# wzhe06/SparrowRecSys

Hardware: AMD Instinct MI355X
Metric: ctr_samples_per_sec (higher is better)
Workload: dtype f32

## Files before the change

sparrowrecsys_amd/csrc/host_setup_common.h:

```cpp
struct DinVariant { int kc, hc, max_t; };
const DinVariant kDinVariants[] = {{2, 2, 64}, {1, 2, 64}};

int fold_first_dense(sprk_engine* h, DevPlan* dp) {
    if (!h->tune.tile_fold) return SPRK_OK;
    if (dp->n_ops < 1) return SPRK_OK;
    DevOp& op = dp->ops[0];
    if (op.kind != SPRK_OP_DENSE || op.src_buf != 0 || op.dst_buf == 0 || op.N > 512) return SPRK_OK;
    const int lo0 = op.src_off, hi0 = op.src_off + op.K;
    auto used_elsewhere = [&](int a, int b) {
        std::vector<char> live(b - a, 1);
        auto reads = [&](int s0, int s1) {
            for (int c = (s0 > a ? s0 : a); c < (s1 < b ? s1 : b); ++c) if (live[c - a]) return true;
            return false;
        };
        auto writes = [&](int s0, int s1) { for (int c = (s0 > a ? s0 : a); c < (s1 < b ? s1 : b); ++c) live[c - a] = 0; };
        for (int i = 1; i < dp->n_ops; ++i) {
            const DevOp& o = dp->ops[i];
            if (o.src_buf == 0) {
                if (o.kind == SPRK_OP_PAIR_DOT) {
                    for (int p = 0; p < dp->n_pairs; ++p)
                        if (reads(dp->pair_a[p], dp->pair_a[p] + o.K) || reads(dp->pair_b[p], dp->pair_b[p] + o.K)) return true;
                } else if (o.kind == SPRK_OP_FM_SUMSQ) {
                    if (reads(o.src_off, o.src_off + (o.groups - 1) * o.group_stride + o.K)) return true;
                } else if (reads(o.src_off, o.src_off + o.K)) {
// ... 60 lines not shown
        std::vector<DevSeg> plain, acc;
        for (int i = 0; i < dp->n_segs; ++i) (dp->segs[i].kind == SEG_ROWS_ACC ? acc : plain).push_back(dp->segs[i]);
        int k = 0;
        for (const DevSeg& g : plain) dp->segs[k++] = g;
        for (const DevSeg& g : acc) dp->segs[k++] = g;
        dp->n_acc = (int)acc.size();
        h->n_acc_folded = dp->n_acc;
    }
    op.W = wcopy + (lo - lo0);
    op.src_off = lo;
    op.K = hi - lo;
    op.acc_init = 1;
    return SPRK_OK;
}

int wide_dynamic_range(const float* rows, long long nrows, int row_floats, int ncols, float mx, bool* wide) {
    *wide = false;
    const bool guard_on = g_finalize_tune ? g_finalize_tune->half_range_guard : SprkTuning::from_env().half_range_guard;
    if (!guard_on || !(mx > 0.f) || nrows <= 0) return SPRK_OK;
    DevScratch<unsigned long long> d_cnt;
    HIP_TRY(d_cnt.alloc(2));
    HIP_TRY(hipMemset(d_cnt.p, 0, 2 * sizeof(unsigned long long)));
    long long blocks = (nrows * ncols + 255) / 256;
    if (blocks > 8192) blocks = 8192;
    hipLaunchKernelGGL(k_v2_count_small, dim3((unsigned)blocks), dim3(256), 0, 0, rows, nrows, row_floats, ncols, ldexpf(mx, -20), d_cnt.p);
    HIP_TRY(hipGetLastError());
    unsigned long long cnt[2] = {0, 0};
    HIP_TRY(hipMemcpy(cnt, d_cnt.p, sizeof(cnt), hipMemcpyDeviceToHost));
    *wide = cnt[0] * 1024ull > cnt[1];
    return SPRK_OK;
}

inline float absmax_nan(float m, float v) { const float a = fabsf(v); return (a > m || a != a) ? a : m; }
bool wide_dynamic_range_host(const float* v, size_t n, float mx) {
    const bool guard_on = g_finalize_tune ? g_finalize_tune->half_range_guard : SprkTuning::from_env().half_range_guard;
    if (!guard_on || !(mx > 0.f)) return false;
    const float thresh = ldexpf(mx, -20);
    unsigned long long small = 0, nz = 0;
    for (size_t i = 0; i < n; ++i) {
        const float a = fabsf(v[i]);
// ... 13 lines not shown

struct AbsmaxJob { const float* x; long long rows; int row_floats, ncols; unsigned grid; int slot; };
int device_absmax(const std::vector<AbsmaxJob>& jobs, float* mx, int n_out) {
    DevScratch<unsigned> d_max;
    HIP_TRY(d_max.alloc(n_out));
    HIP_TRY(hipMemset(d_max.p, 0, n_out * sizeof(unsigned)));
    for (const AbsmaxJob& j : jobs)
        hipLaunchKernelGGL(k_v2_absmax, dim3(j.grid), dim3(256), 0, 0, j.x, j.rows, j.row_floats, j.ncols, d_max.p + j.slot);
    HIP_TRY(hipGetLastError());
    static_assert(sizeof(unsigned) == sizeof(float), "k_v2_absmax keeps float bits in an unsigned word");
    HIP_TRY(hipMemcpy(mx, d_max.p, n_out * sizeof(float), hipMemcpyDeviceToHost));
    return SPRK_OK;
}
unsigned absmax_grid(long long n, long long cap) { const long long b = (n + 255) / 256; return (unsigned)(b < cap ? b : cap); }

int static_scale(const std::vector<AbsmaxJob>& tabs, float* scale, float* mx_out = nullptr) {
    *scale = 0.f;
    float mx = 0.f;
    SPRK_TRY(device_absmax(tabs, &mx, 1));
    if (mx_out) *mx_out = mx;
    if (!(mx < 3.0e38f)) return SPRK_OK;
    for (const AbsmaxJob& t : tabs) {
        bool wide = false;
        SPRK_TRY(wide_dynamic_range(t.x, t.rows, t.row_floats, t.ncols, mx, &wide));
        if (wide) return SPRK_OK;
    }
    *scale = pow2_scale(mx);
    return SPRK_OK;
}
float static_scale_host(const float* v, size_t n) {
    float mx = 0.f;
    for (size_t i = 0; i < n; ++i) mx = absmax_nan(mx, v[i]);
    if (!(mx < 3.0e38f) || wide_dynamic_range_host(v, n, mx)) return 0.f;
    return pow2_scale(mx);
}

int make_dyn_fragments(sprk_engine* h, const float* W, int ld, int N, int K, float** frag, float* w_scale_out, int kvalid = -1) {
    *frag = nullptr;
    if (kvalid < 0) kvalid = K;
// ... 15 lines not shown
```

sparrowrecsys_amd/csrc/host_setup_v2.h:

```cpp
constexpr int V2_WAVES = 8;
struct V2Variant {
    int g_emb, kpc, h0c, h1c;
    size_t lds_bytes;
    void (*pack)(const V2Args, float*);
};
#define V2_LDS(G_EMB, DV, KPC, H0C, H1C, FOLD) \
    (sizeof(float) * (V2Lds<G_EMB, DV, KPC, H0C, H1C, FOLD>::total_pad + V2_WAVES * V2Lds<G_EMB, DV, KPC, H0C, H1C, FOLD>::stage_floats))
#define V2_VARIANT(G_EMB) {G_EMB, 1, 2, 1, V2_LDS(G_EMB, 4, 1, 2, 1, true), &k_v2_pack_image<G_EMB, 4, 1, 2, 1, true>}
const V2Variant kV2Variants[] = {
    V2_VARIANT(6),
    V2_VARIANT(4),
    V2_VARIANT(5), V2_VARIANT(3), V2_VARIANT(2),
};

struct V2JVariant {
    int g_big, njf, kpc;
    bool half;
    V2JKernel fn;
    V2JManyKernel fn_many;
    V2JManyTabKernel fn_many_tab;
};
#define V2J_VARIANT(G_BIG, NJF, HALF) \
    {G_BIG, NJF, 1, HALF, &k_deepfm_v2_joint<G_BIG, NJF, 1, 2, 1, V2_WAVES, HALF>, &k_deepfm_v2_joint_many<G_BIG, NJF, 1, 2, 1, V2_WAVES, HALF>, \
     &k_deepfm_v2_joint_many_tab<G_BIG, NJF, 1, 2, 1, V2_WAVES, HALF>}
// ... 140 lines not shown
}

int setup_v2_joint(sprk_engine* h) {
    const V2Variant& vv = kV2Variants[h->v2_variant];
    if (vv.kpc != 1 || vv.h0c != 2 || vv.h1c != 1 || !h->tune.v2_joint) return SPRK_OK;
    const int KP = 16, H0 = 32, G = vv.g_emb;
    int big[V2_MAX_FIELDS], nbig = 0, jf[V2_MAX_FIELDS], njf = 0;
    for (int g = 0; g < G; ++g) {
        const long long v1 = (long long)h->v2run.vocab[g] + 1;
        if (v1 <= 32 && njf < V2J_MAX_JF) jf[njf++] = g;
        else big[nbig++] = g;
    }
    if (njf < 1 || nbig < 1 || nbig > 3) return SPRK_OK;
    bool half = h->tune.v2_half;
    float p_scale = 1.f, w_scale = 1.f;
    if (half) {
        std::vector<AbsmaxJob> rows_jobs;
        for (int b = 0; b < nbig; ++b) {
            const long long rows = (long long)h->v2run.vocab[big[b]] + 1;
            rows_jobs.push_back({h->v2_folded + (size_t)h->v2run.rowbase[big[b]] * (KP + 16), rows, KP + 16, KP, absmax_grid(rows * KP, 8192), 0});
        }
        SPRK_TRY(static_scale(rows_jobs, &p_scale));
        if (p_scale != 0.f) SPRK_TRY(static_scale({{h->v2.W0, (long long)H0, (G + 1) * KP, (G + 1) * KP, 8, 0}}, &w_scale));
        if (p_scale == 0.f || w_scale == 0.f) { half = false; p_scale = w_scale = 1.f; }
    }
    int variant = -1;
    for (size_t v = 0; v < sizeof(kV2JVariants) / sizeof(kV2JVariants[0]); ++v)
        if (kV2JVariants[v].g_big == nbig && kV2JVariants[v].njf == njf && kV2JVariants[v].half == half) variant = (int)v;
    if (variant < 0) return SPRK_OK;
    V2JRun& r = h->v2j_run;
    memset(&r, 0, sizeof(r));
    r.F = h->v2run.F; r.ND = h->v2run.ND; r.n_num = h->v2run.n_num;
    r.h0w = h->v2run.h0w; r.fo_bias = h->v2run.fo_bias; r.head_bias = h->v2run.head_bias;
    for (int b = 0; b < nbig; ++b) {
        r.big_col[b] = h->v2run.col[big[b]]; r.big_vocab[b] = h->v2run.vocab[big[b]];
        r.big_rowbase[b] = h->v2run.rowbase[big[b]]; r.big_grp[b] = big[b];
    }
    size_t small_floats = 0;
    for (int f = 0; f < njf; ++f) {
// ... 9 lines not shown
    for (int f = 0; f < njf; ++f) {
        const int rows = r.j_vocab[f] + 1;
        hipLaunchKernelGGL(k_v2_fold_small, dim3((rows + 3) / 4), dim3(256), 0, 0,
                           h->v2_folded + (size_t)h->v2run.rowbase[jf[f]] * (KP + 16), KP, H0, jf[f], h->v2.W0, (G + 1) * KP,
                           h->v2.b0, f == 0 ? 1 : 0, h->v2j_tab + r.s_off[f], rows);
    }
    if (half)
        hipLaunchKernelGGL(k_v2j_fold_num, dim3(8), dim3(256), 0, 0, h->v2.W0, (G + 1) * KP, G * KP, h->v2.Wp[G], h->v2.ldp_num,
                           h->v2.bp[G], h->v2.n_num, KP, H0, h->v2j_tab + r.wf_off, h->v2j_tab + r.s_off[0], r.j_vocab[0] + 1);
    HIP_TRY(hipGetLastError());
    HIP_TRY(hipDeviceSynchronize());
    r.small_floats = (int)small_floats;
    r.tab0 = h->v2_folded;
    r.small = h->v2j_tab;
    r.w_scale = w_scale; r.unscale_h = 1.f / (p_scale * w_scale); r.unscale_s = 1.f / p_scale;
    if (half) {
        size_t big_rows = 0;
        for (int b = 0; b < nbig; ++b) big_rows += (size_t)r.big_vocab[b] + 1;
        if (big_rows * (KP + 16) * sizeof(float) >= ((size_t)1 << 32)) return fail(SPRK_EINVAL, "split rows exceed 32-bit offsets");
        SPRK_TRY(table_alloc(h, &h->v2j_big, big_rows * (KP + 16) * sizeof(float)));
        h->derived_bytes += big_rows * (KP + 16) * sizeof(float);
        size_t base = 0;
        for (int b = 0; b < nbig; ++b) {
            const long long rows = (long long)r.big_vocab[b] + 1;
            long long nb = (rows * 8 + 255) / 256;
            if (nb > 65536) nb = 65536;
            hipLaunchKernelGGL(k_v2_split_rows, dim3((unsigned)nb), dim3(256), 0, 0,
                               h->v2_folded + (size_t)r.big_rowbase[b] * (KP + 16), h->v2j_big + base * (KP + 16), rows, p_scale);
            r.big_rowbase[b] = (unsigned)base;
            base += (size_t)rows;
        }
        HIP_TRY(hipGetLastError());
        HIP_TRY(hipDeviceSynchronize());
        r.tab0 = h->v2j_big;
    }
    h->v2j_lds_bytes = vv.lds_bytes + small_floats * sizeof(float);
    SPRK_TRY(set_max_lds(kV2JVariants[variant].fn, h->v2j_lds_bytes));
    SPRK_TRY(set_max_lds(kV2JVariants[variant].fn_many, h->v2j_lds_bytes));
    SPRK_TRY(set_max_lds(kV2JVariants[variant].fn_many_tab, h->v2j_lds_bytes));
    h->v2j_variant = variant;
    if (half && h->tune.v2j_one) {
        for (size_t v = 0; v < sizeof(kV2J1Variants) / sizeof(kV2J1Variants[0]); ++v) {
            const V2J1Variant& ov = kV2J1Variants[v];
// ... 55 lines not shown
```

sparrowrecsys_amd/csrc/k_chain_v2j.h:

```cpp

#define V2J_MAX_BIG 4
#define V2J_MAX_JF 3
#define V2J_SS 52

struct V2JRun {
    int F, ND, n_num;
    int big_col[V2J_MAX_BIG];
    int big_vocab[V2J_MAX_BIG];
    unsigned big_rowbase[V2J_MAX_BIG];
    int big_grp[V2J_MAX_BIG];
    int j_col[V2J_MAX_JF];
    int j_vocab[V2J_MAX_JF];
    int s_off[V2J_MAX_JF];
    int small_floats;
    int wf_off;
    const float* tab0;
    const float* small;
    float h0w, fo_bias, head_bias;
    int flags;
    float w_scale, unscale_h, unscale_s;
};

#define V2J_MB 64
struct V2JMany {
    const int* ids[V2J_MB];
    const float* dense[V2J_MB];
    float* out[V2J_MB];
    int n;
    int ntpb;
};
struct V2JBatch {
    const int* ids;
    const float* dense;
    float* out;
    void* pad_;
};
struct V2JManyTab {
    const V2JBatch* batch;
    int n;
    int ntpb;
};
struct V2JOne {};
__device__ __forceinline__ const int* v2j_ids(const V2JMany& m, int b) { return m.ids[b]; }
__device__ __forceinline__ const float* v2j_dense(const V2JMany& m, int b) { return m.dense[b]; }
__device__ __forceinline__ float* v2j_out(const V2JMany& m, int b) { return m.out[b]; }
typedef const __attribute__((address_space(4))) V2JBatch* V2JBatchCP;
__device__ __forceinline__ const int* v2j_ids(const V2JManyTab& m, int b) { return ((V2JBatchCP)(uintptr_t)m.batch + b)->ids; }
__device__ __forceinline__ const float* v2j_dense(const V2JManyTab& m, int b) { return ((V2JBatchCP)(uintptr_t)m.batch + b)->dense; }
__device__ __forceinline__ float* v2j_out(const V2JManyTab& m, int b) { return ((V2JBatchCP)(uintptr_t)m.batch + b)->out; }

__device__ __forceinline__ void split_half4(f32x4 w, float scale, f16x4& hi, f16x4& lo) {
#pragma unroll
    for (int j = 0; j < 4; ++j) {
        const float x = w[j] * scale;
        const _Float16 h = (_Float16)x;
        hi[j] = h;
        lo[j] = (_Float16)(x - (float)h);
    }
}

static __global__ __launch_bounds__(256) void k_v2_absmax(const float* __restrict__ rows, long long nrows, int row_floats,
                                                   int ncols, unsigned* __restrict__ out) {
    float m = 0.f;
    const long long total = nrows * ncols;
    for (long long i = (long long)blockIdx.x * 256 + threadIdx.x; i < total; i += (long long)gridDim.x * 256) {
// ... 8 lines not shown
static __global__ __launch_bounds__(256) void k_v2_count_small(const float* __restrict__ rows, long long nrows, int row_floats, int ncols,
                                                        float thresh, unsigned long long* __restrict__ out) {
    unsigned small = 0, nz = 0;
    const long long total = nrows * ncols;
    for (long long i = (long long)blockIdx.x * 256 + threadIdx.x; i < total; i += (long long)gridDim.x * 256) {
        const long long v = i / ncols;
        const int c = (int)(i - v * ncols);
        const float a = fabsf(rows[v * row_floats + c]);
        nz += a > 0.f;
        small += (a > 0.f && a < thresh);
    }
    for (int d = 32; d >= 1; d >>= 1) { small += __shfl_xor(small, d); nz += __shfl_xor(nz, d); }
    if ((threadIdx.x & 63) == 0) { atomicAdd(out, (unsigned long long)small); atomicAdd(out + 1, (unsigned long long)nz); }
}
static __global__ __launch_bounds__(256) void k_v2_split_rows(const float* __restrict__ src, float* __restrict__ dst,
                                                       long long nrows, float scale) {
    const long long total = nrows * 8;
    for (long long i = (long long)blockIdx.x * 256 + threadIdx.x; i < total; i += (long long)gridDim.x * 256) {
        const long long v = i >> 3;
        const int pc = (int)(i & 7);
        const f32x4 in = ld4(src + v * 32 + 4 * pc);
        if (pc < 4) {
            f16x4 hi, lo;
            split_half4(in, scale, hi, lo);
            f16x8 o = {hi[0], hi[1], hi[2], hi[3], lo[0], lo[1], lo[2], lo[3]};
            *reinterpret_cast<f16x8*>(dst + v * 32 + 4 * pc) = o;
        } else {
            st4(dst + v * 32 + 4 * pc, in);
        }
    }
}

static __global__ __launch_bounds__(256) void k_v2_fold_small(const float* __restrict__ folded, int KP, int H0, int grp,
                                                       const float* __restrict__ W0, int ldw0,
                                                       const float* __restrict__ b0, int add_b0,
                                                       float* __restrict__ out, int rows) {
    const int FS = KP + 16;
    for (int v = blockIdx.x * 4 + (threadIdx.x >> 6); v < rows; v += gridDim.x * 4) {
        const int col = threadIdx.x & 63;
        const float* prow = folded + (size_t)v * FS;
        float acc = 0.f;
        if (col < KP) {
            acc = prow[col];
        } else if (col < KP + H0) {
// ... 44 lines not shown
    int so[NJF];
    f32x4 xn;
    float w1a;
    float* dst;
};

template <int G_BIG, int NJF, int KPC, int H0C, int H1C, int WAVES, bool HALF, class Many>
__device__ __forceinline__ void v2j_body(const V2JRun& A, const int* __restrict__ ids, const float* __restrict__ dense,
                                         float* __restrict__ out, int B, int* __restrict__ err,
                                         const float* __restrict__ image, const Many* __restrict__ Mp) {
    constexpr bool MB = !std::is_same<Many, V2JOne>::value;
    constexpr int G_EMB = G_BIG + NJF;
    using LD = V2Lds<G_EMB, 4, KPC, H0C, H1C, true>;
    using Set = V2JSet<G_BIG, NJF>;
    constexpr int KP = LD::KP, H0 = H0C * 16;
    constexpr unsigned RB = (KP + 16) * 4;
    static_assert(KP + H0 + 1 <= V2J_SS, "small-field row layout");
    constexpr int NKR = HALF ? 1 : (G_BIG + 1) * KPC;
    static_assert(KPC == 1, "row layout: one 16-float chunk of projections per field");
    static_assert(G_BIG >= 1 && G_BIG <= 3 && NJF >= 1 && NJF <= V2J_MAX_JF, "field split");
    const int tid = threadIdx.x;
    const int lane = tid & 63;
    const int wave = __builtin_amdgcn_readfirstlane(tid >> 6);
    const int r = lane & 15, q = lane >> 4;
    const f32x4 zero = f32x4{0.f, 0.f, 0.f, 0.f};
    int m_ntpb = 0, ntasks = (B + 15) >> 4;
    if constexpr (MB) { m_ntpb = Mp->ntpb; ntasks = Mp->n * m_ntpb; }
    const int task_stride = gridDim.x * WAVES;
    const int wave_global = blockIdx.x * WAVES + wave;
    auto batch_of = [&](int tk) -> int {
        if constexpr (MB) return __builtin_amdgcn_readfirstlane(tk / m_ntpb);
// ... 54 lines not shown
            const float* nrow = stage + 128 + r * A.ND;
            const int c0 = 4 * q, last = A.n_num - 1;
            if constexpr (HALF) {
                S.xn.x = nrow[min(q, last)];
                S.xn.y = nrow[min(q + 4, last)];
            } else {
                S.xn.x = nrow[min(c0 + 0, last)];
                S.xn.y = nrow[min(c0 + 1, last)];
                S.xn.z = nrow[min(c0 + 2, last)];
                S.xn.w = nrow[min(c0 + 3, last)];
            }
        }
        const char* tb = reinterpret_cast<const char*>(A.tab0);
#pragma unroll
        for (int b = 0; b < G_BIG; ++b) S.x[b] = *reinterpret_cast<const f32x4*>(tb + (sid[b] * RB + 16u * q));
        {
            unsigned s0 = sid[0] * RB, s1 = sid[G_BIG > 1 ? 1 : 0] * RB, s2 = sid[G_BIG > 2 ? 2 : 0] * RB;
            asm("" : "+v"(s0), "+v"(s1), "+v"(s2));
            unsigned so = s0;
            if (G_BIG > 1) so = q == 1 ? s1 : so;
            if (G_BIG > 2) so = q == 2 ? s2 : so;
            S.w1a = *reinterpret_cast<const float*>(tb + (so + 4u * KP));
        }
        {
            float* out_b;
            if constexpr (MB) {
                out_b = v2j_out(*Mp, b);
                asm("" : "+s"(out_b));
            } else {
                out_b = out;
            }
            const int m = tk * 16 + r;
            S.dst = (q == 0 && m < B) ? out_b + m : nullptr;
        }
    };

    f32x4 rW0[H0C][NKR], rW1[H1C][H0C];
    f32x4 rwn[KPC], rbpn[KPC], rb1[H1C], rhfm[KPC], rhd[H1C];
    f32x4 rfn = zero;
    float rwn8[2] = {0.f, 0.f}, rfn8[2] = {0.f, 0.f}, rwf[H0C][2];
    f16x8 hWa[HALF ? G_BIG : 1][H0C], hWb[HALF ? G_BIG : 1][H0C];
    f16x8 hSel = {0, 0, 0, 0, 0, 0, 0, 0};
    auto load_weights = [&]() {
        const float* w0r = wq + LD::off_w0 + r * LD::S0;
#pragma unroll
        for (int n0 = 0; n0 < H0C; ++n0) {
            if constexpr (HALF) {
                rwf[n0][0] = small_s[A.wf_off + (n0 * 16 + r) * 8 + q];
                rwf[n0][1] = small_s[A.wf_off + (n0 * 16 + r) * 8 + q + 4];
            } else {
                rW0[n0][0] = ld4(w0r + n0 * 16 * LD::S0 + 16 * G_EMB);
            }
#pragma unroll
            for (int b = 0; b < G_BIG; ++b) {
                const f32x4 w = ld4(w0r + n0 * 16 * LD::S0 + 16 * A.big_grp[b]);
// ... 18 lines not shown
            rb1[n1] = ld4(wq + LD::off_b1 + n1 * 16);
            rhd[n1] = ld4(wq + LD::off_hd + n1 * 16);
        }
#pragma unroll
        for (int nb = 0; nb < KPC; ++nb) {
            rwn[nb] = ld4(wq + LD::off_wn + (nb * 16 + r) * LD::SN);
            rbpn[nb] = ld4(wq + LD::off_bp + G_EMB * KP + nb * 16);
            rhfm[nb] = ld4(wq + LD::off_hfm + nb * 16);
        }
        rfn = ld4(smem + LD::off_fn + 4 * (q & 1));
        if constexpr (HALF) {
            rwn8[0] = smem[LD::off_wn + r * LD::SN + q];
            rwn8[1] = smem[LD::off_wn + r * LD::SN + q + 4];
            rfn8[0] = smem[LD::off_fn + q];
            rfn8[1] = smem[LD::off_fn + q + 4];
        }
    };

    auto compute = [&](const Set& S) -> float {
#pragma clang fp contract(off)
        const f32x4 pnum = S.xn;
        f32x4 pn;
        if constexpr (HALF) {
            const f32x4 e = __builtin_amdgcn_mfma_f32_16x16x4f32(rwn8[0], pnum.x, rbpn[0], 0, 0, 0);
            const f32x4 o = __builtin_amdgcn_mfma_f32_16x16x4f32(rwn8[1], pnum.y, zero, 0, 0, 0);
            pn = e + o;
        } else {
            f32x4 e = rbpn[0], o = zero;
            e = __builtin_amdgcn_mfma_f32_16x16x4f32(rwn[0].x, pnum.x, e, 0, 0, 0);
            o = __builtin_amdgcn_mfma_f32_16x16x4f32(rwn[0].y, pnum.y, o, 0, 0, 0);
            e = __builtin_amdgcn_mfma_f32_16x16x4f32(rwn[0].z, pnum.z, e, 0, 0, 0);
            o = __builtin_amdgcn_mfma_f32_16x16x4f32(rwn[0].w, pnum.w, o, 0, 0, 0);
            pn = e + o;
        }
        float zz = ((q < G_BIG) ? S.w1a : 0.f) + (HALF ? __builtin_fmaf(rfn8[1], pnum.y, rfn8[0] * pnum.x) : ((q < 2) ? dot4f(rfn, pnum) : 0.f));
        f32x4 sp = ld4(small_s + S.so[0] + 4 * q), sq[H0C];
#pragma unroll
        for (int n0 = 0; n0 < H0C; ++n0) sq[n0] = ld4(small_s + S.so[0] + KP + 16 * n0 + 4 * q);
        float ssc = small_s[S.so[0] + KP + H0];
#pragma unroll
        for (int f = 1; f < NJF; ++f) {
            sp += ld4(small_s + S.so[f] + 4 * q);
#pragma unroll
            for (int n0 = 0; n0 < H0C; ++n0) sq[n0] += ld4(small_s + S.so[f] + KP + 16 * n0 + 4 * q);
            ssc += small_s[S.so[f] + KP + H0];
        }
        zz += (q == 3) ? ssc : 0.f;
        f32x4 hA[H0C], hB[H0C];
#pragma unroll
        for (int n0 = 0; n0 < H0C; ++n0) { hA[n0] = sq[n0]; hB[n0] = zero; }
        f32x4 s = sp + pn;
        if constexpr (HALF) {
            f32x4 aFa[H0C], aFb[H0C], aS = zero;
#pragma unroll
            for (int n0 = 0; n0 < H0C; ++n0) { aFa[n0] = zero; aFb[n0] = zero; }
            __builtin_amdgcn_sched_barrier(0);
#pragma unroll
            for (int b = 0; b < G_BIG; ++b) {
                const f16x8 xb = __builtin_bit_cast(f16x8, S.x[b]);
#pragma unroll
                for (int n0 = 0; n0 < H0C; ++n0) aFa[n0] = __builtin_amdgcn_mfma_f32_16x16x32_f16(hWa[b][n0], xb, aFa[n0], 0, 0, 0);
                aS = __builtin_amdgcn_mfma_f32_16x16x32_f16(hSel, xb, aS, 0, 0, 0);
#pragma unroll
                for (int n0 = 0; n0 < H0C; ++n0) aFb[n0] = __builtin_amdgcn_mfma_f32_16x16x32_f16(hWb[b][n0], xb, aFb[n0], 0, 0, 0);
                __builtin_amdgcn_sched_barrier(0);
            }
#pragma unroll
            for (int st = 0; st < 2; ++st)
#pragma unroll
                for (int n0 = 0; n0 < H0C; ++n0)
                    hA[n0] = __builtin_amdgcn_mfma_f32_16x16x4f32(rwf[n0][st], st ? pnum.y : pnum.x, hA[n0], 0, 0, 0);
            s = fma4s(aS, A.unscale_s, s);
#pragma unroll
            for (int n0 = 0; n0 < H0C; ++n0) hB[n0] = (aFa[n0] + aFb[n0]) * A.unscale_h;
        } else {
#pragma unroll
            for (int b = 0; b < G_BIG; ++b) s += S.x[b];
            __builtin_amdgcn_sched_barrier(0);
#pragma unroll
// ... 40 lines not shown
    };

    Set SA, SB;
    f32x4 rawA = zero, rawB = zero;
    int tA = wave_global, tB = wave_global + task_stride;
    int nA = 0, nB = 0;
    if (ntasks > 0) {
        nA = ld_raw(clampt(tA), rawA);
        nB = ld_raw(clampt(tB), rawB);
    }
#pragma unroll 1
    for (int c = wave; c < LD::total_pad / 256; c += WAVES) lds_dma16(image + c * 256 + lane * 4, smem + c * 256);
#pragma unroll 1
    for (int c = wave; c < A.small_floats / 256; c += WAVES) lds_dma16(A.small + c * 256 + lane * 4, smem + LD::total_pad + WAVES * LD::stage_floats + c * 256);
    const bool two = tA < ntasks && ntasks <= 2 * task_stride;
    constexpr int NG = G_BIG + 1;
    static_assert(NG < 16, "s_waitcnt immediate below encodes vmcnt < 16");
    if (two) {
        gather(tA, nA, rawA, SA);
        __builtin_amdgcn_s_waitcnt(0x0F70 | NG);
    } else {
        __builtin_amdgcn_s_waitcnt(0x0F70);
        if (tA < ntasks) {
            gather(tA, nA, rawA, SA);
            nA = ld_raw(clampt(tA + 2 * task_stride), rawA);
            gather(clampt(tB), nB, rawB, SB);
            nB = ld_raw(clampt(tB + 2 * task_stride), rawB);
        }
    }
    __builtin_amdgcn_s_barrier();
    load_weights();
// ... 39 lines not shown
```

sparrowrecsys_amd/csrc/k_chain_v2j1.h:

```cpp

#define V2J1_WAVES 16
#define V2J1_WAVES_HOIST 8
#define V2J1_WAVES_OF(HOIST, G_BIG) (((HOIST) && (G_BIG) >= 3) ? V2J1_WAVES_HOIST : V2J1_WAVES)
#define V2J1_MAX_TASKS 16384

template <int G_BIG>
struct V2J1Lds {
    static constexpr int off_frag = 0;
    static constexpr int S1 = 36;
    static constexpr int off_w1 = off_frag + G_BIG * 2 * 256;
    static constexpr int off_b1 = off_w1 + 16 * S1;
    static constexpr int off_hd = off_b1 + 16;
    static constexpr int off_bpn = off_hd + 16;
    static constexpr int off_hfm = off_bpn + 16;
    static constexpr int off_wn8 = off_hfm + 16;
    static constexpr int off_fn8 = off_wn8 + 128;
    static constexpr int total = off_fn8 + 8;
    static constexpr int total_pad = (total + 255) & ~255;
};

static __global__ __launch_bounds__(256) void k_v2j1_pack_image(const V2Args A, const V2JRun R, int g_big, int G, float* __restrict__ img) {
    const int tid = threadIdx.x;
    const int off_w1 = g_big * 2 * 256, off_b1 = off_w1 + 16 * 36, off_hd = off_b1 + 16, off_bpn = off_hd + 16,
              off_hfm = off_bpn + 16, off_wn8 = off_hfm + 16, off_fn8 = off_wn8 + 128, total_pad = (off_fn8 + 8 + 255) & ~255;
// ... 13 lines not shown
        img[off_hd + tid] = tid < A.n_hdeep ? A.hdeep[tid] : 0.f;
        img[off_bpn + tid] = A.bp[G - 1][tid];
        img[off_hfm + tid] = tid < A.n_hfm ? A.hfm[tid] : 0.f;
    }
    if (tid < 128) img[off_wn8 + tid] = (tid & 7) < A.n_num ? A.Wp[G - 1][(size_t)(tid >> 3) * A.ldp_num + (tid & 7)] : 0.f;
    if (tid < 8) img[off_fn8 + tid] = tid < A.n_num ? A.h0w * A.fo_num_w[tid] : 0.f;
}

template <int G_BIG, int NJF, bool HOIST = false>
__global__ __launch_bounds__(V2J1_WAVES_OF(HOIST, G_BIG) * 64, 4) void k_deepfm_v2_joint1(const V2JRun A, const int* __restrict__ ids,
                                                                       const float* __restrict__ dense, float* __restrict__ out, int B,
                                                                       int* __restrict__ err, const float* __restrict__ image) {
#pragma clang fp contract(off)
    using LD = V2J1Lds<G_BIG>;
    constexpr int WAVES = V2J1_WAVES_OF(HOIST, G_BIG), KP = 16, H0C = 2;
    constexpr unsigned RB = (KP + 16) * 4;
    static_assert(G_BIG >= 1 && G_BIG <= 3 && NJF >= 1 && NJF <= V2J_MAX_JF, "field split");
    const int tid = threadIdx.x;
    const int lane = tid & 63;
    const int wave = __builtin_amdgcn_readfirstlane(tid >> 6);
    const int r = lane & 15, q = lane >> 4;
    const f32x4 zero = f32x4{0.f, 0.f, 0.f, 0.f};
    const int ntasks = (B + 15) >> 4;
    const int tk = blockIdx.x * WAVES + wave;
    const bool work = tk < ntasks;
    const float* small_s = smem + LD::total_pad;
    float* stage = smem + LD::total_pad + A.small_floats + wave * 256;
    const bool fast = work && !(A.flags & 1) && tk * 16 + 16 <= B;

    f32x4 raw = zero;
    if (fast) {
// ... 29 lines not shown
                wa[b][n0] = f16x8{t[0], t[1], t[2], t[3], t[0], t[1], t[2], t[3]};
                wb[b][n0] = f16x8{t[4], t[5], t[6], t[7], t[4], t[5], t[6], t[7]};
            }
        const int d = r - 4 * q;
        const unsigned lo01 = d == 0 ? 0x00003C00u : d == 1 ? 0x3C000000u : 0u, lo23 = d == 2 ? 0x00003C00u : d == 3 ? 0x3C000000u : 0u;
        typedef unsigned u32x4 __attribute__((ext_vector_type(4)));
        hSel = __builtin_bit_cast(f16x8, u32x4{lo01, lo23, lo01, lo23});
    };
    if constexpr (HOIST) {
        read_frags();
        expand_frags();
        __builtin_amdgcn_sched_barrier(0);
    }
    f32x4 x[G_BIG];
    int so[NJF];
    float xn0 = 0.f, xn1 = 0.f, w1a = 0.f;
    bool bad = false;
#pragma unroll
    for (int b = 0; b < G_BIG; ++b) x[b] = zero;
#pragma unroll
    for (int f = 0; f < NJF; ++f) so[f] = 0;
    {
        if (fast) {
            const bool isid = lane < 32;
            const int j = isid ? lane : lane - 32;
            const int n4 = 4 * (isid ? A.F : A.ND);
            if (j < n4) st4(stage + (isid ? 0 : 128) + 4 * j, raw);
        } else {
            stage_task_slow(stage, ids, dense, A.F, A.ND, tk, B, lane);
        }
        const int* sid_row = reinterpret_cast<const int*>(stage) + r * A.F;
// ... 7 lines not shown
#pragma unroll
        for (int f = 0; f < NJF; ++f) {
            const int id = sid_row[A.j_col[f]];
            bad |= (unsigned)(id + 1) > (unsigned)A.j_vocab[f];
            so[f] = A.s_off[f] + (int)min((unsigned)id, (unsigned)A.j_vocab[f]) * V2J_SS;
        }
        {
            const float* nrow = stage + 128 + r * A.ND;
            const int last = A.n_num - 1;
            xn0 = nrow[min(q, last)];
            xn1 = nrow[min(q + 4, last)];
        }
        const char* tb = reinterpret_cast<const char*>(A.tab0);
#pragma unroll
        for (int b = 0; b < G_BIG; ++b) x[b] = *reinterpret_cast<const f32x4*>(tb + (sid[b] * RB + 16u * q));
        {
            unsigned s0 = sid[0] * RB, s1 = sid[G_BIG > 1 ? 1 : 0] * RB, s2 = sid[G_BIG > 2 ? 2 : 0] * RB;
            asm("" : "+v"(s0), "+v"(s1), "+v"(s2));
            unsigned sx = s0;
            if (G_BIG > 1) sx = q == 1 ? s1 : sx;
            if (G_BIG > 2) sx = q == 2 ? s2 : sx;
            w1a = *reinterpret_cast<const float*>(tb + (sx + 4u * KP));
        }
    }

    const float* vq = smem + 4 * q;
    const f32x4 rbpn = ld4(vq + LD::off_bpn);
    const float rwn8a = smem[LD::off_wn8 + r * 8 + q], rwn8b = smem[LD::off_wn8 + r * 8 + q + 4];
    const float rfn8a = smem[LD::off_fn8 + q], rfn8b = smem[LD::off_fn8 + q + 4];
    f32x4 sp = ld4(small_s + so[0] + 4 * q), sq[H0C];
#pragma unroll
    for (int n0 = 0; n0 < H0C; ++n0) sq[n0] = ld4(small_s + so[0] + KP + 16 * n0 + 4 * q);
    float ssc = small_s[so[0] + KP + 32];
#pragma unroll
    for (int f = 1; f < NJF; ++f) {
        sp += ld4(small_s + so[f] + 4 * q);
#pragma unroll
        for (int n0 = 0; n0 < H0C; ++n0) sq[n0] += ld4(small_s + so[f] + KP + 16 * n0 + 4 * q);
// ... 5 lines not shown
        const float* wf = small_s + A.wf_off + r * 8 + q;
#pragma unroll
        for (int n0 = 0; n0 < H0C; ++n0) { rwf[n0][0] = wf[n0 * 128]; rwf[n0][1] = wf[n0 * 128 + 4]; }
    }
    f32x4 rW1[H0C];
#pragma unroll
    for (int j = 0; j < H0C; ++j) rW1[j] = ld4(vq + LD::off_w1 + r * LD::S1 + 16 * j);
    const f32x4 rb1 = ld4(vq + LD::off_b1), rhd = ld4(vq + LD::off_hd), rhfm = ld4(vq + LD::off_hfm);
    f32x4 pn;
    {
        const f32x4 e = __builtin_amdgcn_mfma_f32_16x16x4f32(rwn8a, xn0, rbpn, 0, 0, 0);
        const f32x4 o = __builtin_amdgcn_mfma_f32_16x16x4f32(rwn8b, xn1, zero, 0, 0, 0);
        pn = e + o;
    }
    const float zz_num = __builtin_fmaf(rfn8b, xn1, rfn8a * xn0);
    float zz = 0.f;
    if constexpr (HOIST) {
        zz = ((q < G_BIG) ? w1a : 0.f) + zz_num;
        zz += (q == 3) ? ssc : 0.f;
    }
    f32x4 hA[H0C], hB[H0C];
#pragma unroll
    for (int n0 = 0; n0 < H0C; ++n0) hA[n0] = sq[n0];
#pragma unroll
    for (int st = 0; st < 2; ++st)
#pragma unroll
        for (int n0 = 0; n0 < H0C; ++n0) hA[n0] = __builtin_amdgcn_mfma_f32_16x16x4f32(rwf[n0][st], st ? xn1 : xn0, hA[n0], 0, 0, 0);
    f32x4 s = sp + pn;
    __builtin_amdgcn_sched_barrier(0);
    {
        f32x4 aFa[H0C], aFb[H0C], aS = zero;
#pragma unroll
        for (int n0 = 0; n0 < H0C; ++n0) { aFa[n0] = zero; aFb[n0] = zero; }
#pragma unroll
        for (int b = 0; b < G_BIG; ++b) {
            const f16x8 xb = __builtin_bit_cast(f16x8, x[b]);
#pragma unroll
            for (int n0 = 0; n0 < H0C; ++n0) aFa[n0] = __builtin_amdgcn_mfma_f32_16x16x32_f16(wa[b][n0], xb, aFa[n0], 0, 0, 0);
            aS = __builtin_amdgcn_mfma_f32_16x16x32_f16(hSel, xb, aS, 0, 0, 0);
#pragma unroll
            for (int n0 = 0; n0 < H0C; ++n0) aFb[n0] = __builtin_amdgcn_mfma_f32_16x16x32_f16(wb[b][n0], xb, aFb[n0], 0, 0, 0);
            __builtin_amdgcn_sched_barrier(0);
        }
        s = fma4s(aS, A.unscale_s, s);
#pragma unroll
        for (int n0 = 0; n0 < H0C; ++n0) hB[n0] = (aFa[n0] + aFb[n0]) * A.unscale_h;
    }
    f32x4 h0[H0C];
#pragma unroll
    for (int n0 = 0; n0 < H0C; ++n0) h0[n0] = relu4_fast(hA[n0] + hB[n0]);
    float z = dot4f(rhfm, sq_diff4(s, pn));
    {
        f32x4 e = rb1, o = zero;
#pragma unroll
        for (int j = 0; j < H0C; ++j) {
            e = __builtin_amdgcn_mfma_f32_16x16x4f32(rW1[j].x, h0[j].x, e, 0, 0, 0);
            o = __builtin_amdgcn_mfma_f32_16x16x4f32(rW1[j].y, h0[j].y, o, 0, 0, 0);
            e = __builtin_amdgcn_mfma_f32_16x16x4f32(rW1[j].z, h0[j].z, e, 0, 0, 0);
            o = __builtin_amdgcn_mfma_f32_16x16x4f32(rW1[j].w, h0[j].w, o, 0, 0, 0);
        }
        z += dot4f(rhd, relu4_fast(e + o));
    }
    if constexpr (!HOIST) {
        zz = ((q < G_BIG) ? w1a : 0.f) + zz_num;
        zz += (q == 3) ? ssc : 0.f;
    }
    z += zz;
    z = rows4_sum(z);
    const float score = sigmoidf_fast(z + A.h0w * A.fo_bias + A.head_bias);
    const int m = tk * 16 + r;
    if (q == 0 && m < B) out[m] = score;
    if (__ballot(bad) != 0 && lane == 0) atomicOr(err, 1);
}
```

Baseline: 17.61 billion.

## Pack per-row scalar into low-half mantissa bits to shrink big-field rows

The half-precision split rows for the big embedding fields drop from KP+16 floats to KP floats. The per-row scalar (the w1a term) is quantized to a 32-bit fixed-point value and its bytes are hidden in spare low bits of the f16 low-part words. The hi part is floor-rounded so the lo remainders stay small enough to free those bits. This removes the separate scalar gather load per row and halves the row stride, which cuts memory traffic in the gather-bound kernel. In exchange it adds bit unpacking in the kernel, loses some precision in the lo part and the scalar, and adds a new range check that can turn half mode off.

```diff
diff --git a/sparrowrecsys_amd/csrc/host_setup_common.h b/sparrowrecsys_amd/csrc/host_setup_common.h
--- a/sparrowrecsys_amd/csrc/host_setup_common.h
+++ b/sparrowrecsys_amd/csrc/host_setup_common.h
@@ -98,7 +98,7 @@
     return SPRK_OK;
 }
 
-int wide_dynamic_range(const float* rows, long long nrows, int row_floats, int ncols, float mx, bool* wide) {
+int wide_dynamic_range(const float* rows, long long nrows, int row_floats, int ncols, float mx, bool* wide, int below_exp = -20) {
     *wide = false;
     const bool guard_on = g_finalize_tune ? g_finalize_tune->half_range_guard : SprkTuning::from_env().half_range_guard;
     if (!guard_on || !(mx > 0.f) || nrows <= 0) return SPRK_OK;
@@ -107,7 +107,7 @@
     HIP_TRY(hipMemset(d_cnt.p, 0, 2 * sizeof(unsigned long long)));
     long long blocks = (nrows * ncols + 255) / 256;
     if (blocks > 8192) blocks = 8192;
-    hipLaunchKernelGGL(k_v2_count_small, dim3((unsigned)blocks), dim3(256), 0, 0, rows, nrows, row_floats, ncols, ldexpf(mx, -20), d_cnt.p);
+    hipLaunchKernelGGL(k_v2_count_small, dim3((unsigned)blocks), dim3(256), 0, 0, rows, nrows, row_floats, ncols, ldexpf(mx, below_exp), d_cnt.p);
     HIP_TRY(hipGetLastError());
     unsigned long long cnt[2] = {0, 0};
     HIP_TRY(hipMemcpy(cnt, d_cnt.p, sizeof(cnt), hipMemcpyDeviceToHost));
@@ -151,7 +151,7 @@
 }
 unsigned absmax_grid(long long n, long long cap) { const long long b = (n + 255) / 256; return (unsigned)(b < cap ? b : cap); }
 
-int static_scale(const std::vector<AbsmaxJob>& tabs, float* scale, float* mx_out = nullptr) {
+int static_scale(const std::vector<AbsmaxJob>& tabs, float* scale, float* mx_out = nullptr, int below_exp = -20) {
     *scale = 0.f;
     float mx = 0.f;
     SPRK_TRY(device_absmax(tabs, &mx, 1));
@@ -159,7 +159,7 @@
     if (!(mx < 3.0e38f)) return SPRK_OK;
     for (const AbsmaxJob& t : tabs) {
         bool wide = false;
-        SPRK_TRY(wide_dynamic_range(t.x, t.rows, t.row_floats, t.ncols, mx, &wide));
+        SPRK_TRY(wide_dynamic_range(t.x, t.rows, t.row_floats, t.ncols, mx, &wide, below_exp));
         if (wide) return SPRK_OK;
     }
     *scale = pow2_scale(mx);
diff --git a/sparrowrecsys_amd/csrc/host_setup_v2.h b/sparrowrecsys_amd/csrc/host_setup_v2.h
--- a/sparrowrecsys_amd/csrc/host_setup_v2.h
+++ b/sparrowrecsys_amd/csrc/host_setup_v2.h
@@ -178,15 +178,27 @@
     if (njf < 1 || nbig < 1 || nbig > 3) return SPRK_OK;
     bool half = h->tune.v2_half;
     float p_scale = 1.f, w_scale = 1.f;
+    int sk = 0;
     if (half) {
-        std::vector<AbsmaxJob> rows_jobs;
+        std::vector<AbsmaxJob> rows_jobs, scal_jobs;
         for (int b = 0; b < nbig; ++b) {
             const long long rows = (long long)h->v2run.vocab[big[b]] + 1;
-            rows_jobs.push_back({h->v2_folded + (size_t)h->v2run.rowbase[big[b]] * (KP + 16), rows, KP + 16, KP, absmax_grid(rows * KP, 8192), 0});
-        }
-        SPRK_TRY(static_scale(rows_jobs, &p_scale));
+            const float* fr = h->v2_folded + (size_t)h->v2run.rowbase[big[b]] * (KP + 16);
+            rows_jobs.push_back({fr, rows, KP + 16, KP, absmax_grid(rows * KP, 8192), 0});
+            scal_jobs.push_back({fr + KP, rows, KP + 16, 1, absmax_grid(rows, 8192), 0});
+        }
+        SPRK_TRY(static_scale(rows_jobs, &p_scale, nullptr, -16));
+        p_scale *= 1.f / 16.f;
         if (p_scale != 0.f) SPRK_TRY(static_scale({{h->v2.W0, (long long)H0, (G + 1) * KP, (G + 1) * KP, 8, 0}}, &w_scale));
-        if (p_scale == 0.f || w_scale == 0.f) { half = false; p_scale = w_scale = 1.f; }
+        float smx = 0.f;
+        if (p_scale != 0.f && w_scale != 0.f) SPRK_TRY(device_absmax(scal_jobs, &smx, 1));
+        if (smx > 0.f && smx < 3.0e38f) {
+            int e = 0;
+            (void)frexpf(smx, &e);
+            sk = 30 - e;
+            if (sk > 100) sk = 100;
+        }
+        if (p_scale == 0.f || w_scale == 0.f || !(smx > 0.f && smx < 3.0e38f) || (sk < 20 && h->tune.half_range_guard)) { half = false; p_scale = w_scale = 1.f; sk = 0; }
     }
     int variant = -1;
     for (size_t v = 0; v < sizeof(kV2JVariants) / sizeof(kV2JVariants[0]); ++v)
@@ -226,19 +238,20 @@
     r.tab0 = h->v2_folded;
     r.small = h->v2j_tab;
     r.w_scale = w_scale; r.unscale_h = 1.f / (p_scale * w_scale); r.unscale_s = 1.f / p_scale;
+    r.sk = sk;
     if (half) {
         size_t big_rows = 0;
         for (int b = 0; b < nbig; ++b) big_rows += (size_t)r.big_vocab[b] + 1;
-        if (big_rows * (KP + 16) * sizeof(float) >= ((size_t)1 << 32)) return fail(SPRK_EINVAL, "split rows exceed 32-bit offsets");
-        SPRK_TRY(table_alloc(h, &h->v2j_big, big_rows * (KP + 16) * sizeof(float)));
-        h->derived_bytes += big_rows * (KP + 16) * sizeof(float);
+        if (big_rows * KP * sizeof(float) >= ((size_t)1 << 32)) return fail(SPRK_EINVAL, "split rows exceed 32-bit offsets");
+        SPRK_TRY(table_alloc(h, &h->v2j_big, big_rows * KP * sizeof(float)));
+        h->derived_bytes += big_rows * KP * sizeof(float);
         size_t base = 0;
         for (int b = 0; b < nbig; ++b) {
             const long long rows = (long long)r.big_vocab[b] + 1;
-            long long nb = (rows * 8 + 255) / 256;
+            long long nb = (rows * 4 + 255) / 256;
             if (nb > 65536) nb = 65536;
             hipLaunchKernelGGL(k_v2_split_rows, dim3((unsigned)nb), dim3(256), 0, 0,
-                               h->v2_folded + (size_t)r.big_rowbase[b] * (KP + 16), h->v2j_big + base * (KP + 16), rows, p_scale);
+                               h->v2_folded + (size_t)r.big_rowbase[b] * (KP + 16), h->v2j_big + base * KP, rows, p_scale, ldexpf(1.f, sk));
             r.big_rowbase[b] = (unsigned)base;
             base += (size_t)rows;
         }
diff --git a/sparrowrecsys_amd/csrc/k_chain_v2j.h b/sparrowrecsys_amd/csrc/k_chain_v2j.h
--- a/sparrowrecsys_amd/csrc/k_chain_v2j.h
+++ b/sparrowrecsys_amd/csrc/k_chain_v2j.h
@@ -19,6 +19,7 @@
     float h0w, fo_bias, head_bias;
     int flags;
     float w_scale, unscale_h, unscale_s;
+    int sk;
 };
 
 #define V2J_MB 64
@@ -49,6 +50,26 @@
 __device__ __forceinline__ const float* v2j_dense(const V2JManyTab& m, int b) { return ((V2JBatchCP)(uintptr_t)m.batch + b)->dense; }
 __device__ __forceinline__ float* v2j_out(const V2JManyTab& m, int b) { return ((V2JBatchCP)(uintptr_t)m.batch + b)->out; }
 
+#define V2J_LO_MASK 0x3FFF3FFFu
+__device__ __forceinline__ void v2j_pack_lo(unsigned& d2, unsigned& d3, unsigned by) {
+    d2 = (d2 & V2J_LO_MASK) | ((by & 0xC0u) << 24) | ((by & 0x0Cu) << 12);
+    d3 = (d3 & V2J_LO_MASK) | ((by & 0x30u) << 26) | ((by & 0x03u) << 14);
+}
+__device__ __forceinline__ float v2j_scalar_byte(unsigned d2, unsigned d3) {
+    const unsigned t = (d2 & 0xC000C000u) | ((d3 >> 2) & 0x30003000u);
+    return (float)((t | (t << 12)) >> 24);
+}
+__device__ __forceinline__ float v2j_pow2(int e) { return __uint_as_float((unsigned)(127 + e) << 23); }
+__device__ __forceinline__ _Float16 f16_floor(float x) {
+    _Float16 h = (_Float16)x;
+    if ((float)h > x) {
+        unsigned short b = __builtin_bit_cast(unsigned short, h);
+        b = (b & 0x7FFF) == 0 ? (unsigned short)0x8001 : (b & 0x8000) ? (unsigned short)(b + 1) : (unsigned short)(b - 1);
+        h = __builtin_bit_cast(_Float16, b);
+    }
+    return h;
+}
+
 __device__ __forceinline__ void split_half4(f32x4 w, float scale, f16x4& hi, f16x4& lo) {
 #pragma unroll
     for (int j = 0; j < 4; ++j) {
@@ -87,20 +108,28 @@
     if ((threadIdx.x & 63) == 0) { atomicAdd(out, (unsigned long long)small); atomicAdd(out + 1, (unsigned long long)nz); }
 }
 static __global__ __launch_bounds__(256) void k_v2_split_rows(const float* __restrict__ src, float* __restrict__ dst,
-                                                       long long nrows, float scale) {
-    const long long total = nrows * 8;
+                                                       long long nrows, float scale, float sk2) {
+    typedef unsigned u32x4 __attribute__((ext_vector_type(4)));
+    const long long total = nrows * 4;
     for (long long i = (long long)blockIdx.x * 256 + threadIdx.x; i < total; i += (long long)gridDim.x * 256) {
-        const long long v = i >> 3;
-        const int pc = (int)(i & 7);
+        const long long v = i >> 2;
+        const int pc = (int)(i & 3);
         const f32x4 in = ld4(src + v * 32 + 4 * pc);
-        if (pc < 4) {
-            f16x4 hi, lo;
-            split_half4(in, scale, hi, lo);
-            f16x8 o = {hi[0], hi[1], hi[2], hi[3], lo[0], lo[1], lo[2], lo[3]};
-            *reinterpret_cast<f16x8*>(dst + v * 32 + 4 * pc) = o;
-        } else {
-            st4(dst + v * 32 + 4 * pc, in);
-        }
+        const unsigned u = (unsigned)(int)rintf(src[v * 32 + 16] * sk2) + 0x80000000u;
+        f16x8 o;
+#pragma unroll
+        for (int j = 0; j < 4; ++j) {
+            const float x = in[j] * scale;
+            const _Float16 h = f16_floor(x);
+            o[j] = h;
+            o[4 + j] = (_Float16)(x - (float)h);
+        }
+        u32x4 w = __builtin_bit_cast(u32x4, o);
+        unsigned d2 = w.z, d3 = w.w;
+        v2j_pack_lo(d2, d3, (u >> (8 * pc)) & 0xFFu);
+        w.z = d2;
+        w.w = d3;
+        *reinterpret_cast<u32x4*>(dst + v * 16 + 4 * pc) = w;
     }
 }
 
@@ -175,7 +204,7 @@
     using LD = V2Lds<G_EMB, 4, KPC, H0C, H1C, true>;
     using Set = V2JSet<G_BIG, NJF>;
     constexpr int KP = LD::KP, H0 = H0C * 16;
-    constexpr unsigned RB = (KP + 16) * 4;
+    constexpr unsigned RB = HALF ? KP * 4 : (KP + 16) * 4;
     static_assert(KP + H0 + 1 <= V2J_SS, "small-field row layout");
     constexpr int NKR = HALF ? 1 : (G_BIG + 1) * KPC;
     static_assert(KPC == 1, "row layout: one 16-float chunk of projections per field");
@@ -260,7 +289,7 @@
         const char* tb = reinterpret_cast<const char*>(A.tab0);
 #pragma unroll
         for (int b = 0; b < G_BIG; ++b) S.x[b] = *reinterpret_cast<const f32x4*>(tb + (sid[b] * RB + 16u * q));
-        {
+        if constexpr (!HALF) {
             unsigned s0 = sid[0] * RB, s1 = sid[G_BIG > 1 ? 1 : 0] * RB, s2 = sid[G_BIG > 2 ? 2 : 0] * RB;
             asm("" : "+v"(s0), "+v"(s1), "+v"(s2));
             unsigned so = s0;
@@ -285,6 +314,7 @@
     f32x4 rwn[KPC], rbpn[KPC], rb1[H1C], rhfm[KPC], rhd[H1C];
     f32x4 rfn = zero;
     float rwn8[2] = {0.f, 0.f}, rfn8[2] = {0.f, 0.f}, rwf[H0C][2];
+    float rsc = 0.f, rs0 = 0.f;
     f16x8 hWa[HALF ? G_BIG : 1][H0C], hWb[HALF ? G_BIG : 1][H0C];
     f16x8 hSel = {0, 0, 0, 0, 0, 0, 0, 0};
     auto load_weights = [&]() {
@@ -333,6 +363,8 @@
             rwn8[1] = smem[LD::off_wn + r * LD::SN + q + 4];
             rfn8[0] = smem[LD::off_fn + q];
             rfn8[1] = smem[LD::off_fn + q + 4];
+            rsc = v2j_pow2(8 * q - A.sk);
+            rs0 = q == 3 ? -128.f * G_BIG : 0.f;
         }
     };
 
@@ -352,7 +384,7 @@
             o = __builtin_amdgcn_mfma_f32_16x16x4f32(rwn[0].w, pnum.w, o, 0, 0, 0);
             pn = e + o;
         }
-        float zz = ((q < G_BIG) ? S.w1a : 0.f) + (HALF ? __builtin_fmaf(rfn8[1], pnum.y, rfn8[0] * pnum.x) : ((q < 2) ? dot4f(rfn, pnum) : 0.f));
+        float zz = HALF ? __builtin_fmaf(rfn8[1], pnum.y, rfn8[0] * pnum.x) : ((q < G_BIG) ? S.w1a : 0.f) + ((q < 2) ? dot4f(rfn, pnum) : 0.f);
         f32x4 sp = ld4(small_s + S.so[0] + 4 * q), sq[H0C];
 #pragma unroll
         for (int n0 = 0; n0 < H0C; ++n0) sq[n0] = ld4(small_s + S.so[0] + KP + 16 * n0 + 4 * q);
@@ -364,7 +396,7 @@
             for (int n0 = 0; n0 < H0C; ++n0) sq[n0] += ld4(small_s + S.so[f] + KP + 16 * n0 + 4 * q);
             ssc += small_s[S.so[f] + KP + H0];
         }
-        zz += (q == 3) ? ssc : 0.f;
+        if constexpr (!HALF) zz += (q == 3) ? ssc : 0.f;
         f32x4 hA[H0C], hB[H0C];
 #pragma unroll
         for (int n0 = 0; n0 < H0C; ++n0) { hA[n0] = sq[n0]; hB[n0] = zero; }
@@ -374,14 +406,26 @@
 #pragma unroll
             for (int n0 = 0; n0 < H0C; ++n0) { aFa[n0] = zero; aFb[n0] = zero; }
             __builtin_amdgcn_sched_barrier(0);
+            typedef unsigned u32x4 __attribute__((ext_vector_type(4)));
+            f16x8 xb[G_BIG];
+            float sb = rs0;
 #pragma unroll
             for (int b = 0; b < G_BIG; ++b) {
-                const f16x8 xb = __builtin_bit_cast(f16x8, S.x[b]);
-#pragma unroll
-                for (int n0 = 0; n0 < H0C; ++n0) aFa[n0] = __builtin_amdgcn_mfma_f32_16x16x32_f16(hWa[b][n0], xb, aFa[n0], 0, 0, 0);
-                aS = __builtin_amdgcn_mfma_f32_16x16x32_f16(hSel, xb, aS, 0, 0, 0);
-#pragma unroll
-                for (int n0 = 0; n0 < H0C; ++n0) aFb[n0] = __builtin_amdgcn_mfma_f32_16x16x32_f16(hWb[b][n0], xb, aFb[n0], 0, 0, 0);
+                u32x4 w = __builtin_bit_cast(u32x4, S.x[b]);
+                sb += v2j_scalar_byte(w.z, w.w);
+                w.z &= V2J_LO_MASK;
+                w.w &= V2J_LO_MASK;
+                xb[b] = __builtin_bit_cast(f16x8, w);
+            }
+            zz = __builtin_fmaf(sb, rsc, zz);
+            zz += (q == 3) ? ssc : 0.f;
+#pragma unroll
+            for (int b = 0; b < G_BIG; ++b) {
+#pragma unroll
+                for (int n0 = 0; n0 < H0C; ++n0) aFa[n0] = __builtin_amdgcn_mfma_f32_16x16x32_f16(hWa[b][n0], xb[b], aFa[n0], 0, 0, 0);
+                aS = __builtin_amdgcn_mfma_f32_16x16x32_f16(hSel, xb[b], aS, 0, 0, 0);
+#pragma unroll
+                for (int n0 = 0; n0 < H0C; ++n0) aFb[n0] = __builtin_amdgcn_mfma_f32_16x16x32_f16(hWb[b][n0], xb[b], aFb[n0], 0, 0, 0);
                 __builtin_amdgcn_sched_barrier(0);
             }
 #pragma unroll
@@ -452,7 +496,7 @@
 #pragma unroll 1
     for (int c = wave; c < A.small_floats / 256; c += WAVES) lds_dma16(A.small + c * 256 + lane * 4, smem + LD::total_pad + WAVES * LD::stage_floats + c * 256);
     const bool two = tA < ntasks && ntasks <= 2 * task_stride;
-    constexpr int NG = G_BIG + 1;
+    constexpr int NG = HALF ? G_BIG : G_BIG + 1;
     static_assert(NG < 16, "s_waitcnt immediate below encodes vmcnt < 16");
     if (two) {
         gather(tA, nA, rawA, SA);
diff --git a/sparrowrecsys_amd/csrc/k_chain_v2j1.h b/sparrowrecsys_amd/csrc/k_chain_v2j1.h
--- a/sparrowrecsys_amd/csrc/k_chain_v2j1.h
+++ b/sparrowrecsys_amd/csrc/k_chain_v2j1.h
@@ -51,7 +51,7 @@
 #pragma clang fp contract(off)
     using LD = V2J1Lds<G_BIG>;
     constexpr int WAVES = V2J1_WAVES_OF(HOIST, G_BIG), KP = 16, H0C = 2;
-    constexpr unsigned RB = (KP + 16) * 4;
+    constexpr unsigned RB = KP * 4;
     static_assert(G_BIG >= 1 && G_BIG <= 3 && NJF >= 1 && NJF <= V2J_MAX_JF, "field split");
     const int tid = threadIdx.x;
     const int lane = tid & 63;
@@ -111,7 +111,7 @@
     }
     f32x4 x[G_BIG];
     int so[NJF];
-    float xn0 = 0.f, xn1 = 0.f, w1a = 0.f;
+    float xn0 = 0.f, xn1 = 0.f;
     bool bad = false;
 #pragma unroll
     for (int b = 0; b < G_BIG; ++b) x[b] = zero;
@@ -149,14 +149,6 @@
         const char* tb = reinterpret_cast<const char*>(A.tab0);
 #pragma unroll
         for (int b = 0; b < G_BIG; ++b) x[b] = *reinterpret_cast<const f32x4*>(tb + (sid[b] * RB + 16u * q));
-        {
-            unsigned s0 = sid[0] * RB, s1 = sid[G_BIG > 1 ? 1 : 0] * RB, s2 = sid[G_BIG > 2 ? 2 : 0] * RB;
-            asm("" : "+v"(s0), "+v"(s1), "+v"(s2));
-            unsigned sx = s0;
-            if (G_BIG > 1) sx = q == 1 ? s1 : sx;
-            if (G_BIG > 2) sx = q == 2 ? s2 : sx;
-            w1a = *reinterpret_cast<const float*>(tb + (sx + 4u * KP));
-        }
     }
 
     const float* vq = smem + 4 * q;
@@ -192,11 +184,8 @@
         pn = e + o;
     }
     const float zz_num = __builtin_fmaf(rfn8b, xn1, rfn8a * xn0);
-    float zz = 0.f;
-    if constexpr (HOIST) {
-        zz = ((q < G_BIG) ? w1a : 0.f) + zz_num;
-        zz += (q == 3) ? ssc : 0.f;
-    }
+    const float rsc = v2j_pow2(8 * q - A.sk), rs0 = q == 3 ? -128.f * G_BIG : 0.f;
+    float zz;
     f32x4 hA[H0C], hB[H0C];
 #pragma unroll
     for (int n0 = 0; n0 < H0C; ++n0) hA[n0] = sq[n0];
@@ -210,14 +199,26 @@
         f32x4 aFa[H0C], aFb[H0C], aS = zero;
 #pragma unroll
         for (int n0 = 0; n0 < H0C; ++n0) { aFa[n0] = zero; aFb[n0] = zero; }
+        typedef unsigned u32x4 __attribute__((ext_vector_type(4)));
+        f16x8 xb[G_BIG];
+        float sb = rs0;
 #pragma unroll
         for (int b = 0; b < G_BIG; ++b) {
-            const f16x8 xb = __builtin_bit_cast(f16x8, x[b]);
-#pragma unroll
-            for (int n0 = 0; n0 < H0C; ++n0) aFa[n0] = __builtin_amdgcn_mfma_f32_16x16x32_f16(wa[b][n0], xb, aFa[n0], 0, 0, 0);
-            aS = __builtin_amdgcn_mfma_f32_16x16x32_f16(hSel, xb, aS, 0, 0, 0);
-#pragma unroll
-            for (int n0 = 0; n0 < H0C; ++n0) aFb[n0] = __builtin_amdgcn_mfma_f32_16x16x32_f16(wb[b][n0], xb, aFb[n0], 0, 0, 0);
+            u32x4 w = __builtin_bit_cast(u32x4, x[b]);
+            sb += v2j_scalar_byte(w.z, w.w);
+            w.z &= V2J_LO_MASK;
+            w.w &= V2J_LO_MASK;
+            xb[b] = __builtin_bit_cast(f16x8, w);
+        }
+        zz = __builtin_fmaf(sb, rsc, zz_num);
+        zz += (q == 3) ? ssc : 0.f;
+#pragma unroll
+        for (int b = 0; b < G_BIG; ++b) {
+#pragma unroll
+            for (int n0 = 0; n0 < H0C; ++n0) aFa[n0] = __builtin_amdgcn_mfma_f32_16x16x32_f16(wa[b][n0], xb[b], aFa[n0], 0, 0, 0);
+            aS = __builtin_amdgcn_mfma_f32_16x16x32_f16(hSel, xb[b], aS, 0, 0, 0);
+#pragma unroll
+            for (int n0 = 0; n0 < H0C; ++n0) aFb[n0] = __builtin_amdgcn_mfma_f32_16x16x32_f16(wb[b][n0], xb[b], aFb[n0], 0, 0, 0);
             __builtin_amdgcn_sched_barrier(0);
         }
         s = fma4s(aS, A.unscale_s, s);
@@ -238,10 +239,6 @@
             o = __builtin_amdgcn_mfma_f32_16x16x4f32(rW1[j].w, h0[j].w, o, 0, 0, 0);
         }
         z += dot4f(rhd, relu4_fast(e + o));
-    }
-    if constexpr (!HOIST) {
-        zz = ((q < G_BIG) ? w1a : 0.f) + zz_num;
-        zz += (q == 3) ? ssc : 0.f;
     }
     z += zz;
     z = rows4_sum(z);
```

New measurement: 17.11 billion. -2.8%, worse.
